# cv-core/MIT-Driverless-CV-TrainingInfra

Measured on AMD Instinct MI355X. Metric: images/sec training (YOLOv3 416^2 + RektNet 80^2), higher is better.
Workload: dtype bf16; 1 GPU; CVC-YOLOv3 yolo_baseline 416x416 classes=80, train step (fwd+bwd+Adam), 32 img/GPU; global_batch=32, parallelism=dp1, hipgraph=False, optimizer=FusedAdam

## Files before the change

### include/mdcv_hip.h

```cpp
#ifndef MDCV_HIP_H
#define MDCV_HIP_H
#ifdef __cplusplus
extern "C" {
#endif

#define MDCV_OK 0
#define MDCV_EARG (-1)
#define MDCV_F32 0
#define MDCV_BF16 1
#define MDCV_TUNED(dtype, code) (((dtype) & 0xff) | ((code) * 256))
#define MDCV_ACT_NONE 0
#define MDCV_ACT_LEAKY 1
#define MDCV_ACT_RELU 2

int mdcv_conv2d(int dtype, int mode, const void* in, int in_ldc, const void* w_packed, void* out, int out_ldc,
                const float* bias, const void* addsrc, int add_ldc, float* stats_partial,
                int B, int Hin, int Win, int Cin, int Hout, int Wout, int Nout,
                int KH, int KW, int stride, int pad, int dil, void* stream);
int mdcv_conv2d_affine_act(int dtype, const void* in, int in_ldc, const void* w_packed, void* out, int out_ldc, const float* scale,
                           const float* shift, const void* addsrc, int add_ldc, int act, float slope, int B, int Hin, int Win, int Cin,
                           int Hout, int Wout, int Nout, int KH, int KW, int stride, int pad, int dil, void* stream);
int mdcv_conv2d_dgrad_bnsums_rows(int dtype, int B, int Hin, int Win, int Cin, int Hout, int Wout, int Nout, int KH, int KW, int stride,
                                  int pad, int dil, int in_ldc);
int mdcv_conv2d_dgrad_bnsums(int dtype, const void* in, int in_ldc, const void* w_packed, void* out, int out_ldc, const void* addsrc,
                             int add_ldc, int B, int Hin, int Win, int Cin, int Hout, int Wout, int Nout, int KH, int KW, int stride,
                             int pad, int dil, const void* y, int ldy, const float* scale, const float* shift, const float* mean, int act,
                             float slope, float* partial, void* stream);
int mdcv_first_conv_ok(int dtype, int B, int H, int W, int Cin_pad, int Cout_pad, int KH, int KW, int stride, int pad, int dil, int ldx);
int mdcv_first_conv_rows(int B, int H);
int mdcv_first_conv_stats(int dtype, const void* x, int ldx, const void* w_packed, float* partial, int B, int H, int W, void* stream);
int mdcv_first_conv_bn_act(int dtype, const void* x, int ldx, const void* w_packed, const float* scale, const float* shift, int act, float slope,
                           void* y, int ldy, void* z, int ldz, int B, int H, int W, void* stream);
int mdcv_conv2d_dgrad_s2_form_ok(int dtype, int B, int Hin, int Win, int Cin, int Hout, int Wout, int Nout, int KH, int KW, int stride,
                                 int pad, int dil, int in_ldc);
int mdcv_xstats_words(int reps, int C);
int mdcv_xstats_reps(int rows, int C);
int mdcv_conv2d_xstats(int dtype, const void* in, int in_ldc, const void* w_packed, void* out, int out_ldc, const float* bias, void* xacc,
                       int reps, int B, int Hin, int Win, int Cin, int Hout, int Wout, int Nout, int KH, int KW, int stride, int pad, int dil,
                       void* stream);
int mdcv_pw_conv_fwd_xstats(int dtype, const void* y, int ldy, const float* scale, const float* shift, const void* resid, int ldr, int act,
                            float slope, void* z_out, int ldz, const void* w_packed, const float* bias, void* out, int out_ldc, void* xacc,
                            int reps, long long M, int K, int N, void* stream);
int mdcv_bn_act_fwd_xstats(int dtype, const void* y, int ldy, const void* xacc, int reps, double count, const float* gamma, const float* beta,
                           float* running_mean, float* running_var, float momentum, float eps, float* scale, float* shift, float* mean,
                           float* invstd, const void* resid, int ldr, void* out, int ldo, int M, int C, int act, float slope, void* stream);
int mdcv_conv2d_stats_rows(int M);
int mdcv_conv2d_stats_rows_geom(int dtype, int B, int Hout, int Wout, int Cin, int Nout, int KH, int KW, int stride, int pad, int dil,
                                int in_ldc);

int mdcv_conv2d_wgrad_splits(int dtype, int M, int Cout, int Ktot);
int mdcv_conv2d_wgrad_splits_geom(int dtype, int B, int Hin, int Win, int Cin, int Hout, int Wout, int Cout, int KH, int KW, int stride,
                                  int pad, int dil, int dy_ldc, int x_ldc);
int mdcv_conv2d_wgrad(int dtype, const void* dy, int dy_ldc, const void* x, int x_ldc, float* ws, int splits,
                      float* dw_oihw, int accumulate, int B, int Hin, int Win, int Cin, int Cin_real,
                      int Hout, int Wout, int Cout, int Cout_real, int KH, int KW, int stride, int pad, int dil, void* stream);

int mdcv_pack_weights(int dtype, const float* w_oihw, void* w_fwd, void* w_dgrad, int Cout, int Cin, int KH, int KW,
                      int Cout_pad, int Cin_pad, void* stream);

int mdcv_pack_weights_batched(int dtype, const void* table, int nlayers, int max_taps, void* stream);

int mdcv_nchw_to_nhwc(int dtype, const float* src, void* dst, int B, int C, int H, int W, int ldc, int Cpad, void* stream);
int mdcv_nhwc_to_nchw(int dtype, const void* src, int ldc, float* dst, int B, int C, int H, int W, void* stream);

int mdcv_partial_reduce(const float* partial, int rows, int nsums, int C, double* accum, void* stream);
int mdcv_bn_finalize(double* accum, double count, const float* gamma, const float* beta, float* running_mean, float* running_var,
                     float momentum, float eps, float* scale, float* shift, float* mean, float* invstd, int C, void* stream);
int mdcv_bn_eval_coeffs(const float* gamma, const float* beta, const float* running_mean, const float* running_var, float eps,
                        float* scale, float* shift, int C, void* stream);
int mdcv_bn_eval_coeffs_bias(const float* gamma, const float* beta, const float* running_mean, const float* running_var, float eps,
                             const float* conv_bias, float* scale, float* shift, int C, void* stream);
int mdcv_bn_act_fwd(int dtype, const void* y1, int ld1, const float* s1, const float* b1, const void* y2, int ld2, const float* s2,
                    const float* b2, const void* resid, int ldr, void* out, int ldo, int M, int C, int act, float slope, void* stream);
int mdcv_bn_act_bwd_reduce_ws_floats(int dtype, int M, int C, int nsums);
int mdcv_bn_stats_finalize(const float* partial, int rows, double* accum, double count, const float* gamma, const float* beta,
                           float* running_mean, float* running_var, float momentum, float eps, float* scale, float* shift, float* mean,
                           float* invstd, int C, void* stream);
int mdcv_bn_act_bwd_reduce_finalize(int dtype, const void* dout, int ldd, const void* y1, int ld1, const float* s1, const float* b1,
                                    const float* mean1, const float* invstd1, const void* y2, int ld2, const float* s2, const float* b2,
                                    const float* mean2, const float* invstd2, float* partial_ws, int M, int C, int act, float slope,
                                    double count, const float* gamma1, float* dgamma1, float* dbeta1, float* cA1, float* cB1, float* cC1,
                                    const float* gamma2, float* dgamma2, float* dbeta2, float* cA2, float* cB2, float* cC2, void* stream);
int mdcv_bn_bwd_finalize_rows(const float* partial, int rows, int C, double count, const float* gamma, const float* mean,
                              const float* invstd, float* dgamma, float* dbeta, float* cA, float* cB, float* cC, void* stream);
int mdcv_bn_act_bwd_reduce(int dtype, const void* dout, int ldd, const void* y1, int ld1, const float* s1, const float* b1,
                           const float* mean1, const float* invstd1, const void* y2, int ld2, const float* s2, const float* b2,
                           const float* mean2, const float* invstd2, double* accum, float* partial_ws, int M, int C, int act, float slope,
// ... 174 lines not shown
```

### mit-driverless-cv-traininginfra_amd/csrc/bn_fuse.h

```cpp
#pragma once
#include "common.h"

struct EpiArgs { const float* oscale; int act; float slope; };

struct BnFuseArgs {
  const void* y;
  const float* scale; const float* shift; const float* mean;
  float* partial;
  int ldy, act, row_base;
  float slope;
};

__device__ __forceinline__ void lds_only_barrier() { asm volatile("s_waitcnt lgkmcnt(0)\n\ts_barrier" ::: "memory"); }

__device__ __forceinline__ float swap_add16(float u, float v) {
  const auto r = __builtin_amdgcn_permlane16_swap(__builtin_bit_cast(unsigned, u), __builtin_bit_cast(unsigned, v), false, false);
  return __builtin_bit_cast(float, (unsigned)r[0]) + __builtin_bit_cast(float, (unsigned)r[1]);
}
__device__ __forceinline__ float swap_add32(float u, float v) {
  const auto r = __builtin_amdgcn_permlane32_swap(__builtin_bit_cast(unsigned, u), __builtin_bit_cast(unsigned, v), false, false);
  return __builtin_bit_cast(float, (unsigned)r[0]) + __builtin_bit_cast(float, (unsigned)r[1]);
}
template <int CTRL> __device__ __forceinline__ float ror_add(float x) {
  return x + __builtin_bit_cast(float, __builtin_amdgcn_update_dpp(0, __builtin_bit_cast(int, x), CTRL, 0xf, 0xf, false));
}

template <typename T, int BN, int NT>
struct BnFuseAcc {
  static constexpr int VEC = ET<T>::VEC;
  static constexpr int VPRO = BN / VEC;
  static constexpr int RPP = NT / VPRO;
  static_assert(NT % VPRO == 0 && RPP <= 128 && 128 % RPP == 0 && VPRO <= 64, "store-loop geometry");
  float fs[VEC], fb[VEC], fm[VEC], sg[VEC], sx[VEC];

  __device__ __forceinline__ void init(const BnFuseArgs& f, int n0, int Nout) {
#pragma unroll
    for (int e = 0; e < VEC; ++e) {
      const bool ok = f.y && n0 + e < Nout;
      fs[e] = ok ? f.scale[n0 + e] : 0.f; fb[e] = ok ? f.shift[n0 + e] : 0.f; fm[e] = ok ? f.mean[n0 + e] : 0.f;
      sg[e] = 0.f; sx[e] = 0.f;
    }
  }
  __device__ __forceinline__ void add(const BnFuseArgs& f, const float (&dv)[VEC], const uint4& yq) {
    float yv[VEC];
    ET<T>::unpack(yq, yv);
#pragma unroll
    for (int e = 0; e < VEC; ++e) {
      const float pre = __builtin_fmaf(yv[e], fs[e], fb[e]);
      const float g = (f.act != 0 && !(pre > 0.f)) ? dv[e] * f.slope : dv[e];
      sg[e] += g;
      sx[e] += g * (yv[e] - fm[e]);
    }
  }
  static constexpr bool kWaveFold = VEC == 8 && VPRO <= 16;
  static constexpr int WROWS = 64 / VPRO;
  __device__ __forceinline__ void fold_wave(float* ws, int lane) {
    float w[8], x[4];
#pragma unroll
    for (int m = 0; m < 4; ++m) { w[m] = swap_add16(sg[2 * m], sg[2 * m + 1]); w[4 + m] = swap_add16(sx[2 * m], sx[2 * m + 1]); }
#pragma unroll
    for (int n = 0; n < 4; ++n) x[n] = swap_add32(w[2 * n], w[2 * n + 1]);
#pragma unroll
    for (int n = 0; n < 4; ++n) {
      if constexpr (VPRO <= 8) x[n] = ror_add<0x128>(x[n]);
      if constexpr (VPRO <= 4) x[n] = ror_add<0x124>(x[n]);
      if constexpr (VPRO <= 2) x[n] = ror_add<0x122>(x[n]);
    }
    const int rho = lane >> 4, c16 = lane & 15;
    if (c16 < VPRO) {
      float* r0 = ws + c16 * VEC + rho;
      r0[0] = x[0]; r0[4] = x[1]; r0[BN] = x[2]; r0[BN + 4] = x[3];
    }
#pragma unroll
    for (int e = 0; e < VEC; ++e) { sg[e] = 0.f; sx[e] = 0.f; }
  }
  static __device__ __forceinline__ void write_row(const BnFuseArgs& f, const float* ws0, int wstride, int t, int n_tile0, int Nout, int row) {
    const int which = t / BN, c = t - which * BN;
    float tot = 0.f;
#pragma unroll
    for (int wv = 0; wv < NT / 64; ++wv) tot += ws0[wv * wstride + t];
    const int n = n_tile0 + c;
    if (n < Nout) f.partial[(size_t)(f.row_base + row) * 2 * Nout + (size_t)which * Nout + n] = tot;
  }

  __device__ __forceinline__ void flush(const BnFuseArgs& f, float* red, int tid, int n_tile0, int Nout, int row) {
    const int lane = tid & 63, wave = tid >> 6;
    {
#pragma unroll
      for (int off = 32; off >= VPRO; off >>= 1) {
#pragma unroll
        for (int e = 0; e < VEC; ++e) { sg[e] += __shfl_xor(sg[e], off, 64); sx[e] += __shfl_xor(sx[e], off, 64); }
      }
      float tot[2] = {0.f, 0.f};
#pragma unroll
      for (int k = 0; k < 2; ++k) {
        if (lane < VPRO) {
#pragma unroll
          for (int e = 0; e < VEC; ++e) red[wave * BN + lane * VEC + e] = k == 0 ? sg[e] : sx[e];
        }
        lds_only_barrier();
        if (tid < BN) {
#pragma unroll
          for (int w = 0; w < NT / 64; ++w) tot[k] += red[w * BN + tid];
        }
// ... 16 lines not shown
```

### mit-driverless-cv-traininginfra_amd/csrc/conv_igemm.hip

```cpp
#include "conv_gemm.h"
#include "conv_shift.h"
#include "wgrad_gemm.h"
#include "wgrad_shift.h"
#include "wgrad_stream.h"

extern "C" {

static int conv2d_impl(int dtype, int mode, const void* in, int in_ldc, const void* w_packed, void* out, int out_ldc,
                       const float* bias, const void* addsrc, int add_ldc, float* stats_partial,
                       int B, int Hin, int Win, int Cin, int Hout, int Wout, int Nout,
                       int KH, int KW, int stride, int pad, int dil, const BnFuseArgs* fuse, void* stream, const EpiArgs* epi = nullptr,
                       const XAccArgs* xacc = nullptr) {
  if (!in || !w_packed || !out) return MDCV_EARG;
  if (xacc && (mode != 0 || stats_partial || fuse || epi || !xacc->acc || xacc->reps < 1 || (xacc->reps & (xacc->reps - 1)))) return MDCV_EARG;
  if (epi && (mode != 0 || stats_partial || fuse)) return MDCV_EARG;
  if ((Cin & 7) || (Nout & 7) || (in_ldc & 7) || (out_ldc & 7) || (addsrc && (add_ldc & 7))) return MDCV_EARG;
  if (stride != 1 && stride != 2) return MDCV_EARG;
  if (mode != 0 && mode != 1) return MDCV_EARG;
  ConvArgs a;
  a.in = in; a.w = w_packed; a.out = out; a.bias = bias; a.addsrc = addsrc; a.stats = stats_partial;
  a.in_ldc = in_ldc; a.out_ldc = out_ldc; a.add_ldc = add_ldc;
  a.Hin = Hin; a.Win = Win; a.Cin = Cin; a.Hout = Hout; a.Wout = Wout; a.Nout = Nout;
  a.KH = KH; a.KW = KW; a.stride = stride; a.pad = pad; a.dil = dil;
  a.M = B * Hout * Wout; a.Ktot = KH * KW * Cin; a.tiles_n = 0; a.sshift = stride == 2 ? 1 : 0; a.tiles_total = 0; a.xcd_chunk = 0;
// ... 85 lines not shown
                           int Hout, int Wout, int Nout, int KH, int KW, int stride, int pad, int dil, void* stream) {
  MDCV_TUNE_ENTRY(dtype, MDCV_TUNE_CONV);
  if (act < 0 || act > 2) return MDCV_EARG;
  const EpiArgs e{scale, act, slope};
  return conv2d_impl(dtype, 0, in, in_ldc, w_packed, out, out_ldc, shift, addsrc, add_ldc, nullptr, B, Hin, Win, Cin, Hout, Wout, Nout,
                     KH, KW, stride, pad, dil, nullptr, stream, &e);
}

int mdcv_conv2d_dgrad_bnsums_rows(int dtype, int B, int Hin, int Win, int Cin, int Hout, int Wout, int Nout, int KH, int KW, int stride,
                                  int pad, int dil, int in_ldc) {
  MDCV_TUNE_ENTRY(dtype, MDCV_TUNE_CONV);
  const int es = 2;
  if (dtype != MDCV_BF16) return 0;
  if (!conv_operands_small((long long)B * Hin * Win * in_ldc * es, (long long)Nout * KH * KW * Cin * es)) return 0;
  if (Hin == Hout && Win == Wout && mdcv_shift_eligible(dtype, B, Hout, Wout, Cin, Nout, KH, KW, stride, pad, dil, in_ldc))
    return mdcv_shift_stats_rows(B, Hout, Wout, dil, Nout);
  if (stride == 2 && dil == 1 && KH == 3 && KW == 3 && pad == 1 && Hout == 2 * Hin && Wout == 2 * Win && TUNE().conv_variant < 0 &&
      mdcv_shift_s2_dgrad_eligible(dtype, B, Hin, Win, Cin, Nout, in_ldc))
    return mdcv_shift_s2_rows(B, Hin, Win);
  if (stride == 2 && dil == 1) {
    int rows = 0;
    for (int cls = 0; cls < 4; ++cls) {
      const int ph = cls >> 1, pw = cls & 1;
      const int m = B * ((Hout - ph + 1) / 2) * ((Wout - pw + 1) / 2);
      if (m > 0) rows += cdiv(m, 128);
    }
    return rows;
  }
  return cdiv(B * Hout * Wout, 128);
}

int mdcv_conv2d_dgrad_bnsums(int dtype, const void* in, int in_ldc, const void* w_packed, void* out, int out_ldc, const void* addsrc,
                             int add_ldc, int B, int Hin, int Win, int Cin, int Hout, int Wout, int Nout, int KH, int KW, int stride,
                             int pad, int dil, const void* y, int ldy, const float* scale, const float* shift, const float* mean, int act,
                             float slope, float* partial, void* stream) {
  MDCV_TUNE_ENTRY(dtype, MDCV_TUNE_CONV);
  if (!y || !scale || !shift || !mean || !partial || (ldy & 7)) return MDCV_EARG;
  if (mdcv_conv2d_dgrad_bnsums_rows(dtype, B, Hin, Win, Cin, Hout, Wout, Nout, KH, KW, stride, pad, dil, in_ldc) <= 0) return MDCV_EARG;
  BnFuseArgs f;
  f.y = y; f.scale = scale; f.shift = shift; f.mean = mean; f.partial = partial; f.ldy = ldy; f.act = act; f.row_base = 0;
  f.slope = act == 2 ? 0.f : slope;
  return conv2d_impl(dtype, 1, in, in_ldc, w_packed, out, out_ldc, nullptr, addsrc, add_ldc, nullptr, B, Hin, Win, Cin, Hout, Wout, Nout,
                     KH, KW, stride, pad, dil, &f, stream);
}

int mdcv_conv2d_dgrad_s2_form_ok(int dtype, int B, int Hin, int Win, int Cin, int Hout, int Wout, int Nout, int KH, int KW, int stride,
                                 int pad, int dil, int in_ldc) {
  MDCV_TUNE_ENTRY(dtype, MDCV_TUNE_CONV);
  return dtype == MDCV_BF16 && stride == 2 && dil == 1 && KH == 3 && KW == 3 && pad == 1 && Hout == 2 * Hin && Wout == 2 * Win &&
         TUNE().conv_variant < 0 && (long long)B * Hin * Win * in_ldc * 2 < (1LL << 31) &&
         mdcv_shift_s2_dgrad_eligible(dtype, B, Hin, Win, Cin, Nout, in_ldc);
}

int mdcv_conv2d_stats_rows(int M) { return cdiv(M, 128); }
int mdcv_conv2d_stats_rows_geom(int dtype, int B, int Hout, int Wout, int Cin, int Nout, int KH, int KW, int stride, int pad, int dil,
                                int in_ldc) {
  MDCV_TUNE_ENTRY(dtype, MDCV_TUNE_CONV);
  if (mdcv_shift_eligible(dtype, B, Hout, Wout, Cin, Nout, KH, KW, stride, pad, dil, in_ldc)) return mdcv_shift_fwd_stats_rows(B, Hout, Wout, Nout, dil);
  return cdiv(B * Hout * Wout, 128);
}

int mdcv_conv2d_wgrad_splits(int dtype, int M, int Cout, int Ktot) {
  MDCV_TUNE_ENTRY(dtype, MDCV_TUNE_WGRAD);
  const int bp = dtype == MDCV_BF16 ? 128 : 64;
  const int tiles = cdiv(Cout, 128) * cdiv(Ktot, 128);
  const int slots = TUNE().wgrad_slots;
  int s = slots / tiles;
  const int max_s = cdiv(M, bp * 4);
  if (s > max_s) s = max_s;
  if (s < 1) s = 1;
  int pps = cdiv(cdiv(M, s), bp) * bp;
  return cdiv(M, pps);
}

enum WgradFamily { WG_STEM, WG_STREAM, WG_SHIFT, WG_S2, WG_GENERIC };

static bool wgrad_eligible(WgradFamily f, const WgradGeom& g) {
  const int v = TUNE().wgrad_variant;
  if (f == WG_GENERIC) return true;
  if (v == 9 || (v == 10 && f != WG_SHIFT)) return false;
  const bool same = g.Hin == g.Hout && g.Win == g.Wout;
  switch (f) {
    case WG_STEM:
      return same && mdcv_wgrad_stem_eligible(g.dtype, g.B, g.Hout, g.Wout, g.Cin, g.Cout, g.KH, g.KW, g.stride, g.pad, g.dil, g.dy_ldc, g.x_ldc);
    case WG_STREAM:
      return same && mdcv_wgrad_stream_eligible(g.dtype, g.B, g.Hout, g.Wout, g.Cin, g.Cout, g.KH, g.KW, g.stride, g.pad, g.dil, g.dy_ldc, g.x_ldc);
    case WG_S2:
      return mdcv_wgrad_s2_eligible(g.dtype, g.B, g.Hin, g.Win, g.Cin, g.Hout, g.Wout, g.Cout, g.KH, g.KW, g.stride, g.pad, g.dil, g.dy_ldc, g.x_ldc);
    default: break;
  }
  if (!same || !mdcv_wgrad_shift_eligible(g.dtype, g.B, g.Hout, g.Wout, g.Cin, g.Cout, g.KH, g.KW, g.stride, g.pad, g.dil, g.dy_ldc, g.x_ldc)) return false;
  if (v == 8) return true;
  const long long Mq = (long long)g.B * (g.Hout + 1) * (g.Wout + 1);
  const int s = mdcv_wgrad_shift_splits(g.B, g.Hout, g.Wout, g.Cin, g.Cout);
  if (Mq / (64LL * s) >= 128) return true;
  return v == 11 && mdcv_conv2d_wgrad_splits(g.dtype, g.B * g.Hout * g.Wout, g.Cout, g.KH * g.KW * g.Cin) == 1;
}

static int wgrad_family_splits(WgradFamily f, const WgradGeom& g) {
  switch (f) {
    case WG_STEM:   return mdcv_wgrad_stem_splits(g.B, g.Hout, g.Wout);
    case WG_STREAM: return mdcv_wgrad_stream_splits(g.B, g.Hout, g.Wout, g.Cin, g.Cout, g.dil);
    case WG_SHIFT:  return mdcv_wgrad_shift_splits(g.B, g.Hout, g.Wout, g.Cin, g.Cout);
    case WG_S2:     return mdcv_wgrad_s2_splits(g.B, g.Hout, g.Wout, g.Cin, g.Cout);
    default:        return mdcv_conv2d_wgrad_splits(g.dtype, g.B * g.Hout * g.Wout, g.Cout, g.KH * g.KW * g.Cin);
  }
// ... 72 lines not shown
```

### mit-driverless-cv-traininginfra_amd/csrc/conv_shift.h

```cpp
#pragma once
#include <hip/hip_runtime.h>
#include "bn_fuse.h"
#include "exact_acc.h"

struct ShiftArgs {
  const void* in; const void* w; void* out; const float* bias; const void* addsrc; float* stats;
  int in_ldc, out_ldc, add_ldc;
  int B, H, W, Cin, Nout;
  int Wq, Sq, Mq;
  int tiles_n, tiles_total, xcd_chunk;
  int p_base;
  int dil;
  BnFuseArgs fuse;
  EpiArgs epi;
  int t2d, tiles_x, tiles_y, TH;
  int nchunks, wrow, nca;
  XAccArgs xacc;
};

bool mdcv_shift_eligible(int dtype, int B, int H, int W, int Cin, int Nout, int KH, int KW, int stride, int pad, int dil, long long in_ldc);
int mdcv_shift_stats_rows(int B, int H, int W, int dil = 1, int Nout = 128);
int mdcv_shift_fwd_stats_rows(int B, int H, int W, int Nout, int dil = 1);
int mdcv_shift_conv(int mode, const void* in, int in_ldc, const void* w, void* out, int out_ldc, const float* bias, const void* addsrc,
                    int add_ldc, float* stats, int B, int H, int W, int Cin, int Nout, const BnFuseArgs* fuse, hipStream_t st,
                    const EpiArgs* epi = nullptr, int dil = 1, const XAccArgs* xacc = nullptr);
int mdcv_shift_s2_rows(int B, int H, int W);
bool mdcv_shift_s2_dgrad_eligible(int dtype, int B, int H, int W, int Cin, int Nout, long long in_ldc);
```

### mit-driverless-cv-traininginfra_amd/csrc/conv_shift.hip

```cpp
#include "common.h"
#include "conv_shift.h"
#include "bn_fuse.h"

#ifndef MDCV_SHIFT_PART
#define MDCV_SHIFT_PART 0
#endif
#if MDCV_SHIFT_PART == 0
#else
#endif
int mdcv_shift_launch_dgrad(const ShiftArgs& a, hipStream_t st, unsigned in_bytes, unsigned w_bytes);

namespace {

[[maybe_unused]] constexpr int BN = 128;
constexpr int WM = 4;
constexpr unsigned OOB = 0x80000000u;

__device__ __forceinline__ int swz(int row) { return (row >> 1) & 2; }
typedef __attribute__((address_space(3))) void lds_void_t;

#if defined(MDCV_SHIFT_TS) || defined(MDCV_SHIFT_WG)
#include <cstdio>
__device__ long long g_shift_wg[3 * 4096];
#endif
// ... 239 lines not shown
    bf16_t* __restrict__ out3 = reinterpret_cast<bf16_t*>(a.out);
    const bf16_t* __restrict__ add3 = reinterpret_cast<const bf16_t*>(a.addsrc);
    constexpr int VPRO3 = BN / 8;
    static_assert((512 * VPRO3) % (NW * 64) == 0 && (NW * 64) % VPRO3 == 0, "every thread keeps one channel vector");
    using Acc3 = BnFuseAcc<bf16_t, BN, NW * 64>;
    Acc3 fz3;
    const bf16_t* __restrict__ fy3 = reinterpret_cast<const bf16_t*>(a.fuse.y);
    if constexpr (FUSE) fz3.init(a.fuse, tile_n * BN + (tid % VPRO3) * 8, a.Nout);
#pragma unroll
    for (int py = 0; py < 2; ++py) {
#pragma unroll
      for (int px = 0; px < 2; ++px)
#pragma unroll
        for (int i = 0; i < FM; ++i)
#pragma unroll
          for (int j = 0; j < FN; ++j)
#pragma unroll
            for (int rr = 0; rr < 4; ++rr) {
              const int p = wm * TM + i * 16 + (lane >> 4) * 4 + rr, col = wn * TN + j * 16 + (lane & 15);
              const int srow = (p >> 5) * 64 + 2 * (p & 31) + px;
              reinterpret_cast<bf16_t*>(smem + srow * SROW)[col] = f2bf(acc[(2 * py + px) * FM + i][j][rr]);
            }
      __syncthreads();
      long long pixv[VPRO3]; uint4 aq[VPRO3], yq[VPRO3];
      const int cv = tid % VPRO3, n = tile_n * BN + cv * 8;
#pragma unroll
      for (int k = 0; k < VPRO3; ++k) {
        const int srow = (tid + k * NW * 64) / VPRO3;
        const int la = srow >> 6, ox = srow & 63;
        const int Y = 2 * (a0 + la) + py, X = 2 * b0 + ox;
        const bool ok = ox < 2 * (a.Wq - 1) && Y < Ho && X < Wo && n < a.Nout;
        pixv[k] = ok ? ((long long)img * Ho + Y) * Wo + X : -1;
        if (ok) {
          if (add3) aq[k] = *reinterpret_cast<const uint4*>(add3 + pixv[k] * a.add_ldc + n);
          if constexpr (FUSE) yq[k] = *reinterpret_cast<const uint4*>(fy3 + pixv[k] * a.fuse.ldy + n);
        }
      }
#pragma unroll
      for (int k = 0; k < VPRO3; ++k) {
        if (pixv[k] >= 0) {
          const int srow = (tid + k * NW * 64) / VPRO3;
          uint4 d = *reinterpret_cast<const uint4*>(smem + srow * SROW + cv * 16);
          float x[8];
          if (add3 || FUSE) ET<bf16_t>::unpack(d, x);
          if (add3) {
            float y[8];
            ET<bf16_t>::unpack(aq[k], y);
#pragma unroll
            for (int e = 0; e < 8; ++e) x[e] += y[e];
            d = ET<bf16_t>::pack(x);
            if constexpr (FUSE) ET<bf16_t>::unpack(d, x);
          }
          if constexpr (FUSE) {
            fz3.add(a.fuse, x, yq[k]);
          }
          *reinterpret_cast<uint4*>(out3 + pixv[k] * a.out_ldc + n) = d;
        }
      }
      __syncthreads();
    }
    if constexpr (FUSE) {
      static_assert(Acc3::kWaveFold, "bf16, at most 16 channel vectors per pixel");
      float* ws3 = reinterpret_cast<float*>(smem + 512 * SROW);
      fz3.fold_wave(ws3 + wave * 2 * BN, lane);
      lds_only_barrier();
      for (int t = tid; t < 2 * BN; t += NW * 64) Acc3::write_row(a.fuse, ws3, 2 * BN, t, tile_n * BN, a.Nout, tile_m);
    }
    return;
  }
  int* rowpix = reinterpret_cast<int*>(smem + PIX_OFF);
  if (tid < BM) {
    int img, y, x;
    bool ok;
    if (a.t2d) {
      const int tpi = a.tiles_x * a.tiles_y;
      img = tile_m / tpi;
      const int rt = tile_m - img * tpi, ty = rt / a.tiles_x, tx = rt - ty * a.tiles_x;
      const int ly = tid / a.Wq, lx = tid - ly * a.Wq;
      y = ty * a.TH + ly; x = tx * (a.Wq - 2) + lx;
      ok = lx < a.Wq - 2 && ly < a.TH;
    } else {
      const int p = p0 + tid;
      ok = p < a.Mq;
      const int pp = ok ? p : 0;
      img = pp / a.Sq;
      const int rem = pp - img * a.Sq;
      y = rem / a.Wq; x = rem - y * a.Wq;
    }
    ok = ok && y < a.H && x < a.W;
    rowpix[tid] = ok ? (img * a.H + y) * a.W + x : -1;
  }
  const int n0 = tile_n * BN + wn * TN;
  if constexpr (EPI) {
#pragma unroll
    for (int j = 0; j < FN; ++j) {
      const int n = n0 + j * 16 + (lane & 15);
      const float sc = (a.epi.oscale && n < a.Nout) ? a.epi.oscale[n] : 1.f;
      const float bv = (a.bias && n < a.Nout) ? a.bias[n] : 0.f;
      const float sl = a.epi.act == 1 ? a.epi.slope : (a.epi.act == 2 ? 0.f : 1.f);
#pragma unroll
      for (int i = 0; i < FM; ++i)
#pragma unroll
        for (int rr = 0; rr < 4; ++rr) {
          const float v = acc[i][j][rr] * sc + bv;
          acc[i][j][rr] = v > 0.f ? v : v * sl;
        }
    }
// ... 211 lines not shown
  return launch_shift<MODE, BM, 5, 2, BN_>(a, p_base, tiles_m, st, in_bytes, w_bytes);
}

int shift_plan_bm(int Mq, int tiles_n, bool fused, int halo = 0, int bn = 128, bool fwd = false) {
  if (halo > 0 && !fused && 2 * ((256 + halo + 15) / 16) * 1024 + 3 * bn * 64 + 1024 > 80 * 1024) {
    for (int bm = 256; bm >= 128; bm -= 64) {
      const int nca = (bm + halo + 15) / 16;
      if (2 * nca * 1024 + 3 * bn * 64 + 1024 <= 80 * 1024) return bm;
    }
    return 256;
  }
  if (bn == 128 && !fused && fwd && halo <= 110) {
    const int t384 = ((Mq + 383) / 384) * tiles_n;
    if (TUNE().shift_big == 384 || (TUNE().shift_loop == 2 && t384 > 192 && t384 <= 256)) return 384;
  }
  if (TUNE().shift_plan == 1) return 256;
  if (TUNE().shift_plan == 2) return 128;
  const int t256 = ((Mq + 255) / 256) * tiles_n;
  if (t256 <= 128) return 128;
  if (fused || TUNE().shift_plan == 6) return 256;
  const int t192 = ((Mq + 191) / 192) * tiles_n;
  const int c256 = ((t256 + 255) / 256) * 256, c192 = ((t192 + 255) / 256) * 192;
  return c192 < c256 ? 192 : 256;
}

template <int MODE, int BN_>
int launch_shift_mode(const ShiftArgs& a, hipStream_t st, unsigned in_bytes, unsigned w_bytes) {
  if constexpr (MODE == 3) {
    return launch_shift_bm<MODE, 256, BN_>(a, 0, a.Mq / 256, st, in_bytes, w_bytes);
  } else {
  if (a.t2d) return launch_shift_bm<MODE, 256, BN_>(a, 0, a.Mq / 256, st, in_bytes, w_bytes);
  const int bm = shift_plan_bm(a.Mq, a.tiles_n, a.fuse.y != nullptr, 2 * a.dil * (a.Wq + 1), BN_, MODE == 0);
  if constexpr (BN_ == 128 && MODE == 0) {
    if (bm == 384) return launch_shift_bm<MODE, 384, BN_>(a, 0, (a.Mq + 383) / 384, st, in_bytes, w_bytes);
  }
  if (bm == 192) return launch_shift_bm<MODE, 192, BN_>(a, 0, (a.Mq + 191) / 192, st, in_bytes, w_bytes);
  const int big_m = (a.Mq + 255) / 256;
  const int nbig_m = bm == 128 ? 0 : big_m;
  if (nbig_m > 0) {
    const int rc = launch_shift_bm<MODE, 256, BN_>(a, 0, nbig_m, st, in_bytes, w_bytes);
    if (rc) return rc;
  }
  const int p_base = nbig_m * 256;
  if (p_base < a.Mq) return launch_shift_bm<MODE, 128, BN_>(a, p_base, (a.Mq - p_base + 127) / 128, st, in_bytes, w_bytes);
  return MDCV_OK;
  }
}

}

#if MDCV_SHIFT_PART == 1
int mdcv_shift_launch_dgrad(const ShiftArgs& a, hipStream_t st, unsigned in_bytes, unsigned w_bytes) {
  if (a.t2d == 2) {
    if (a.Nout == 32) return launch_shift_mode<3, 32>(a, st, in_bytes, w_bytes);
    if (a.Nout == 64) return launch_shift_mode<3, 64>(a, st, in_bytes, w_bytes);
    return MDCV_EARG;
  }
  if (a.Nout == 32) return launch_shift_mode<1, 32>(a, st, in_bytes, w_bytes);
  if (a.Nout == 64) return launch_shift_mode<1, 64>(a, st, in_bytes, w_bytes);
  if (TUNE().shift_n64_wide && !a.t2d && a.Nout % 64 == 0 && ((a.Mq + 255) / 256) * a.tiles_n <= 128) {
    ShiftArgs b = a;
    b.tiles_n = a.Nout / 64;
    return launch_shift_mode<1, 64>(b, st, in_bytes, w_bytes);
  }
  return launch_shift_mode<1, 128>(a, st, in_bytes, w_bytes);
}
#else
static bool shift_fits_1d(int W, int Nout) {
  return W <= TUNE().shift_wmax || (TUNE().shift_wmax_narrow && Nout <= 64 && W <= TUNE().shift_wmax_narrow) || (TUNE().shift_wmax_n32 && Nout <= 32 && W <= TUNE().shift_wmax_n32);
}
static bool shift_is_2d(int W, int Nout, int dil) { return dil == 1 && TUNE().shift_2d && !shift_fits_1d(W, Nout); }
constexpr int T2D_WQ = 32, T2D_TH = 8;
static long long shift_2d_positions(int B, int H, int W) { return (long long)B * ((H + T2D_TH - 1) / T2D_TH) * ((W + T2D_WQ - 3) / (T2D_WQ - 2)) * 256; }

bool mdcv_shift_eligible(int dtype, int B, int H, int W, int Cin, int Nout, int KH, int KW, int stride, int pad, int dil, long long in_ldc) {
  if (dtype != MDCV_BF16 || KH != 3 || KW != 3 || stride != 1 || pad != dil || (dil != 1 && !(dil == 2 && TUNE().shift_dil2))) return false;
  if (dil == 2 && TUNE().shift_dil2 == 1 && !(Nout <= 64 && Cin >= 64)) return false;
  if ((Cin & 31) || ((Nout & 127) && !(Nout == 64 && TUNE().shift_n64) && !(Nout == 32 && TUNE().shift_n64 == 2))) return false;
  if (H < 8 || W < 8) return false;
  if (!shift_fits_1d(W, Nout) && !(TUNE().shift_2d && dil == 1)) return false;
  if ((long long)B * (H + dil) * (W + dil) + 1024 >= (1LL << 30) || shift_2d_positions(B, H, W) >= (1LL << 30)) return false;
  if ((long long)B * H * W * in_ldc * 2 >= (1LL << 31) || (long long)Nout * 9 * Cin * 2 >= (1LL << 31)) return false;
  return true;
}

bool mdcv_shift_s2_dgrad_eligible(int dtype, int B, int H, int W, int Cin, int Nout, long long in_ldc) {
  if (!TUNE().shift_s2 || dtype != MDCV_BF16 || (Cin & 31) || Cin < 32 || !(Nout == 32 || Nout == 64) || H < 1 || W < 1) return false;
  if ((long long)B * ((H + 7) / 8) * ((W + 30) / 31) * 256 >= (1LL << 30)) return false;
  if ((long long)B * H * W * in_ldc * 2 >= (1LL << 31) || (long long)Nout * 9 * Cin * 2 >= (1LL << 31)) return false;
  return true;
}

int mdcv_shift_s2_rows(int B, int H, int W) { return B * ((H + T2D_TH - 1) / T2D_TH) * ((W + T2D_WQ - 2) / (T2D_WQ - 1)); }

int mdcv_shift_stats_rows(int B, int H, int W, int dil, int Nout) {
  if (shift_is_2d(W, Nout, dil)) return (int)(shift_2d_positions(B, H, W) / 128);
  return (int)(((long long)B * (H + dil) * (W + dil) + 127) / 128);
}
int mdcv_shift_fwd_stats_rows(int B, int H, int W, int Nout, int dil) {
  if (shift_is_2d(W, Nout, dil)) return (int)(shift_2d_positions(B, H, W) / 128);
  const int Mq = B * (H + dil) * (W + dil);
  const int bn = Nout <= 64 ? Nout : BN;
  const int bm = shift_plan_bm(Mq, Nout <= 64 ? 1 : Nout / BN, false, 2 * dil * (W + dil + 1), bn, true);
  return (bm == 192 || bm == 384) ? (Mq + bm - 1) / bm : (Mq + 127) / 128;
}

// ... 58 lines not shown
```

### mit-driverless-cv-traininginfra_amd/csrc/tune.h

```cpp
#pragma once

struct MdcvTune {
  int conv_no_ut = 0;
  int conv_tall_narrow = 256;
  int conv_deep_narrow = 1;
  int conv_deep_small = 8;
  int conv_fuse_narrow = 1;
  int conv_variant = -1;
  int conv_tall_s2 = 1;
  int conv_deep_s2 = 1;
  int conv_s2_allcls = 1;
  int conv_s2_split = 512;
  int conv_s2_split_on = 1;
  int wgrad_slots = 512;
  int wgrad_bna_stages = 2;
  int wgrad_variant = 0;
  int shift_ring = 4;
  int shift_wmax_narrow = 104;
  int shift_wmax_n32 = 0;
  int shift_dil2 = 1;
  int shift_n64 = 2;
  int shift_wmax = 80;
  int shift_loop = 2;
  int shift_2d = 1;
  int shift_big = 0;
  int shift_n64_wide = 1;
  int shift_plan = 0;
  int shift_s2 = 1;
  int pw_bmp = 0;
  int pw_wres = 1;
  int stream_blocks = 0;
  int stream_tiled = 1;
  int stream_light_maxpos = 600000;
  int stream_table = 1;
  int stream_direct = 1;
  int stream_s2 = 1;
  int stream_s2_blocks = 256;
  int stream_s2_depth = 2;
  int stream_s2_lds = 160 * 1024;
  int stream_light_depth = 1;
  int stream_light_blocks = 256;
  int stream_tiled_blocks = 128;
};

extern thread_local const MdcvTune* mdcv_t_tune;
inline const MdcvTune& TUNE() { return *mdcv_t_tune; }

enum { MDCV_TUNE_CONV = 0, MDCV_TUNE_WGRAD = 1, MDCV_TUNE_PW = 2 };

inline void mdcv_tune_shift(MdcvTune& t, int ring) {
  if (ring == 63 || ring == 64) { t.shift_n64_wide = ring - 63; return; }
  if (ring == 29 || ring == 60) { t.shift_s2 = ring == 60; return; }
  if (ring == 27 || ring == 28) { t.shift_2d = ring - 27; return; }
  if (ring >= 200 && ring < 300) { t.shift_big = ring == 201 ? 384 : 0; return; }
  if (ring >= 30 && ring <= 59) { t.shift_loop = ring - 30; return; }
  if (ring == 25 || ring == 26) { t.shift_wmax_n32 = ring == 25 ? 208 : 0; return; }
  if (ring == 23 || ring == 24) { t.shift_wmax_narrow = ring == 23 ? 104 : 0; return; }
  if (ring >= 20 && ring <= 22) { t.shift_dil2 = ring == 20 ? 2 : (ring == 21 ? 0 : 1); return; }
  if (ring >= 17 && ring <= 19) { t.shift_n64 = ring == 17 ? 1 : (ring == 18 ? 0 : 2); return; }
  if (ring >= 14 && ring <= 16) { t.shift_wmax = ring == 14 ? 80 : (ring == 15 ? 62 : 104); return; }
  if (ring >= 7) t.shift_plan = ring - 7;
  else if (ring >= 3 && ring <= 5) t.shift_ring = ring;
}
inline void mdcv_tune_apply_conv(MdcvTune& t, int v) {
  if (v == 0) return;
  if (v <= -3 && v >= -299) { mdcv_tune_shift(t, -v); return; }
  if (v == 93 || v == 92) { t.conv_fuse_narrow = v == 93; return; }
  if (v >= 60 && v < 92) { t.conv_deep_small = v - 60; return; }
  if (v >= 30 && v < 60) { t.conv_deep_narrow = v - 30; return; }
  if (v == 20 || v == 21) { t.conv_deep_s2 = v - 20; return; }
  if (v == 16 || v == 17) { t.conv_s2_allcls = v - 16; return; }
  if (v == 14 || v == 15) { t.conv_s2_split_on = v - 14; return; }
  if (v >= 4000 && v < 6000) { t.conv_s2_split = v - 4000; return; }
  if (v == 18 || v == 19) { t.conv_tall_s2 = v - 18; return; }
  if (v >= 2000 && v < 3000) { t.conv_tall_narrow = v - 2000; return; }
  if (v >= 100) { t.conv_no_ut = 1; v -= 100; }
  if (v >= 1 && v <= 12) t.conv_variant = v - 1;
}
inline void mdcv_tune_apply_wgrad(MdcvTune& t, int v) {
  if (v == 0) return;
  if (v >= 20000 && v < 30000) { t.wgrad_slots = v - 20000; return; }
  if (v >= 35000 && v < 36000) { t.stream_s2_blocks = v - 35000; return; }
  if (v >= 30000 && v < 40000) {
    const int b = v - 30000;
    if (b >= 4001 && b <= 4002) { t.stream_light_depth = b - 4000; return; }
    if (b >= 4012 && b <= 4014) { t.wgrad_bna_stages = b - 4010; return; }
    if (b == 4020 || b == 4021) { t.stream_table = b - 4020; return; }
    if (b == 4050 || b == 4051) { t.stream_direct = b - 4050; return; }
    if (b == 4060 || b == 4061) { t.stream_s2 = b - 4060; return; }
    if (b >= 4071 && b <= 4073) { t.stream_s2_depth = b - 4070; return; }
    if (b >= 4100 && b <= 4260) { t.stream_s2_lds = (b - 4100) * 1024; return; }
    if (b == 2) t.stream_light_maxpos = 600000;
    else if (b == 3) t.stream_light_maxpos = 1 << 30;
    else if (b == 5) t.stream_light_maxpos = 0;
    else if (b >= 3000 && b < 4000) t.stream_light_blocks = b - 3000;
    else t.stream_tiled_blocks = b > 0 ? b : 128;
    return;
  }
  if (v >= 1000) { const int d = (v - 1000) / 100; t.stream_tiled = !(d & 8); t.stream_blocks = ((v - 1000) % 100) * 64; return; }
  t.wgrad_variant = v;
}
inline void mdcv_tune_apply_pw(MdcvTune& t, int v) {
  if (v == 1000 || v == 1001) { t.pw_wres = v - 1000; return; }
  if (v == 64 || v == 32 || v == 16) t.pw_bmp = v;
}

struct TuneScope {
  MdcvTune t;
  const MdcvTune* prev;
  int dtype;
  TuneScope(int dtype_arg, int family) : prev(mdcv_t_tune), dtype(dtype_arg & 0xff) {
    const int code = dtype_arg >> 8;
    if (code != 0) {
      if (family == MDCV_TUNE_CONV) mdcv_tune_apply_conv(t, code);
      else if (family == MDCV_TUNE_WGRAD) mdcv_tune_apply_wgrad(t, code);
      else mdcv_tune_apply_pw(t, code);
      mdcv_t_tune = &t;
    }
  }
// ... 7 lines not shown
```

Baseline: 2501 images/sec.

## Add persistent stride-2 shift dgrad kernel with cross-tile prefetch

```diff
diff --git a/include/mdcv_hip.h b/include/mdcv_hip.h
--- a/include/mdcv_hip.h
+++ b/include/mdcv_hip.h
@@ -33,6 +33,7 @@
                            void* y, int ldy, void* z, int ldz, int B, int H, int W, void* stream);
 int mdcv_conv2d_dgrad_s2_form_ok(int dtype, int B, int Hin, int Win, int Cin, int Hout, int Wout, int Nout, int KH, int KW, int stride,
                                  int pad, int dil, int in_ldc);
+int mdcv_conv2d_dgrad_s2_persistent(int dtype, int Nout);
 int mdcv_xstats_words(int reps, int C);
 int mdcv_xstats_reps(int rows, int C);
 int mdcv_conv2d_xstats(int dtype, const void* in, int in_ldc, const void* w_packed, void* out, int out_ldc, const float* bias, void* xacc,
diff --git a/mit-driverless-cv-traininginfra_amd/csrc/bn_fuse.h b/mit-driverless-cv-traininginfra_amd/csrc/bn_fuse.h
--- a/mit-driverless-cv-traininginfra_amd/csrc/bn_fuse.h
+++ b/mit-driverless-cv-traininginfra_amd/csrc/bn_fuse.h
@@ -50,6 +50,17 @@
       const float g = (f.act != 0 && !(pre > 0.f)) ? dv[e] * f.slope : dv[e];
       sg[e] += g;
       sx[e] += g * (yv[e] - fm[e]);
+    }
+  }
+  __device__ __forceinline__ void add_fma(const BnFuseArgs& f, const float (&dv)[VEC], const uint4& yq) {
+    float yv[VEC];
+    ET<T>::unpack(yq, yv);
+#pragma unroll
+    for (int e = 0; e < VEC; ++e) {
+      const float pre = __builtin_fmaf(yv[e], fs[e], fb[e]);
+      const float g = (f.act != 0 && !(pre > 0.f)) ? dv[e] * f.slope : dv[e];
+      sg[e] += g;
+      sx[e] = __builtin_fmaf(g, yv[e] - fm[e], sx[e]);
     }
   }
   static constexpr bool kWaveFold = VEC == 8 && VPRO <= 16;
diff --git a/mit-driverless-cv-traininginfra_amd/csrc/conv_igemm.hip b/mit-driverless-cv-traininginfra_amd/csrc/conv_igemm.hip
--- a/mit-driverless-cv-traininginfra_amd/csrc/conv_igemm.hip
+++ b/mit-driverless-cv-traininginfra_amd/csrc/conv_igemm.hip
@@ -161,6 +161,11 @@
          mdcv_shift_s2_dgrad_eligible(dtype, B, Hin, Win, Cin, Nout, in_ldc);
 }
 
+int mdcv_conv2d_dgrad_s2_persistent(int dtype, int Nout) {
+  MDCV_TUNE_ENTRY(dtype, MDCV_TUNE_CONV);
+  return dtype == MDCV_BF16 && TUNE().shift_s2 && mdcv_shift_s2_persistent(Nout) ? 1 : 0;
+}
+
 int mdcv_conv2d_stats_rows(int M) { return cdiv(M, 128); }
 int mdcv_conv2d_stats_rows_geom(int dtype, int B, int Hout, int Wout, int Cin, int Nout, int KH, int KW, int stride, int pad, int dil,
                                 int in_ldc) {
diff --git a/mit-driverless-cv-traininginfra_amd/csrc/conv_shift.h b/mit-driverless-cv-traininginfra_amd/csrc/conv_shift.h
--- a/mit-driverless-cv-traininginfra_amd/csrc/conv_shift.h
+++ b/mit-driverless-cv-traininginfra_amd/csrc/conv_shift.h
@@ -26,3 +26,5 @@
                     const EpiArgs* epi = nullptr, int dil = 1, const XAccArgs* xacc = nullptr);
 int mdcv_shift_s2_rows(int B, int H, int W);
 bool mdcv_shift_s2_dgrad_eligible(int dtype, int B, int H, int W, int Cin, int Nout, long long in_ldc);
+bool mdcv_shift_s2_persistent(int Nout);
+int mdcv_shift_s2p_launch(const ShiftArgs& a, hipStream_t st, unsigned in_bytes, unsigned w_bytes);
diff --git a/mit-driverless-cv-traininginfra_amd/csrc/conv_shift.hip b/mit-driverless-cv-traininginfra_amd/csrc/conv_shift.hip
--- a/mit-driverless-cv-traininginfra_amd/csrc/conv_shift.hip
+++ b/mit-driverless-cv-traininginfra_amd/csrc/conv_shift.hip
@@ -315,7 +315,7 @@
             if constexpr (FUSE) ET<bf16_t>::unpack(d, x);
           }
           if constexpr (FUSE) {
-            fz3.add(a.fuse, x, yq[k]);
+            fz3.add_fma(a.fuse, x, yq[k]);
           }
           *reinterpret_cast<uint4*>(out3 + pixv[k] * a.out_ldc + n) = d;
         }
@@ -633,6 +633,7 @@
 #if MDCV_SHIFT_PART == 1
 int mdcv_shift_launch_dgrad(const ShiftArgs& a, hipStream_t st, unsigned in_bytes, unsigned w_bytes) {
   if (a.t2d == 2) {
+    if (mdcv_shift_s2_persistent(a.Nout)) return mdcv_shift_s2p_launch(a, st, in_bytes, w_bytes);
     if (a.Nout == 32) return launch_shift_mode<3, 32>(a, st, in_bytes, w_bytes);
     if (a.Nout == 64) return launch_shift_mode<3, 64>(a, st, in_bytes, w_bytes);
     return MDCV_EARG;
diff --git a/mit-driverless-cv-traininginfra_amd/csrc/conv_shift_s2p.hip b/mit-driverless-cv-traininginfra_amd/csrc/conv_shift_s2p.hip
--- /dev/null
+++ b/mit-driverless-cv-traininginfra_amd/csrc/conv_shift_s2p.hip
@@ -0,0 +1,331 @@
+#include "common.h"
+#include "conv_shift.h"
+#include "bn_fuse.h"
+
+namespace {
+
+constexpr unsigned OOB = 0x80000000u;
+__device__ __forceinline__ int swz(int row) { return (row >> 1) & 2; }
+typedef __attribute__((address_space(3))) void lds_void_t;
+template <int N> __device__ __forceinline__ void wait_vm() { asm volatile("s_waitcnt vmcnt(%0)" ::"n"(N) : "memory"); }
+template <int N> __device__ __forceinline__ void wait_vm_reads_done() { asm volatile("s_waitcnt vmcnt(%0) lgkmcnt(0)" ::"n"(N) : "memory"); }
+
+template <int BN> struct S2pGeom {
+  static constexpr int NW = 8, WN = 2, NPA = 3, NCA = 21;
+  static constexpr int BTILE = BN * 64, SROW = BN * 2 + 16, ABYTES = NCA * 1024;
+  static constexpr int STG = 512 * SROW;
+  static constexpr int EXTRA = ((STG - ABYTES + 1023) / 1024) * 1024;
+  static constexpr int A1OFF = ABYTES + EXTRA, BBASE = A1OFF + ABYTES, SINK = BBASE + 3 * BTILE;
+  static constexpr int WS_OFF = SINK + 1024, TAB_OFF = WS_OFF + NW * 2 * BN * 4, LDS = TAB_OFF + 3 * BN * 4;
+  static constexpr int WPC = BN == 32 ? 2 : 1;
+  static_assert(EXTRA >= 0 && A1OFF >= STG && EXTRA + ABYTES >= STG, "the staging area fits beside the buffer the prefetch lands in");
+};
+
+}
+
+template <int BN_, bool FUSE>
+__global__ __launch_bounds__(512) __attribute__((amdgpu_waves_per_eu(BN_ == 32 ? 4 : 2, BN_ == 32 ? 4 : 2)))
+void mdcv_shift_s2p_kernel(ShiftArgs a, unsigned in_bytes, unsigned w_bytes, int lanes, int grid) {
+  using G = S2pGeom<BN_>;
+  constexpr int BN = BN_, BTILE = G::BTILE, SROW = G::SROW, NW = G::NW, WN = G::WN, NPA = G::NPA, ABYTES = G::ABYTES;
+  constexpr int TN = BN / WN, FN = TN / 16, TM = 64, FM = 4, LA = 2, BRING = 3;
+  extern __shared__ __attribute__((aligned(1024))) unsigned char smem[];
+
+  const int x = (int)blockIdx.x % lanes, jx = (int)blockIdx.x / lanes, nx = (grid - x + lanes - 1) / lanes;
+  const int hi = min((x + 1) * a.xcd_chunk, a.tiles_total);
+  int t = x * a.xcd_chunk + jx;
+  if (t >= hi) return;
+
+  const int tid = threadIdx.x;
+  const int wave = __builtin_amdgcn_readfirstlane(tid >> 6);
+  const int wm = wave / WN, wn = wave % WN;
+  const int tpi = a.tiles_x * a.tiles_y;
+
+  const __amdgpu_buffer_rsrc_t rin = __builtin_amdgcn_make_buffer_rsrc(const_cast<void*>(a.in), 0, in_bytes, 0x00020000);
+  const __amdgpu_buffer_rsrc_t rw = __builtin_amdgcn_make_buffer_rsrc(const_cast<void*>(a.w), 0, w_bytes, 0x00020000);
+#define S2P_ABUF(B) ((B) ? G::A1OFF : 0)
+#define S2P_ISSUE_A(RS, AVO, CHUNK, BUF)                                                                               \
+  do {                                                                                                                \
+    const int base__ = S2P_ABUF(BUF);                                                                                 \
+    const int so__ = (CHUNK) * 64;                                                                                    \
+    _Pragma("unroll") for (int k = 0; k < NPA; ++k) {                                                                 \
+      const int ch__ = wave + k * NW;              \
+      __builtin_amdgcn_raw_ptr_buffer_load_lds(RS, (lds_void_t*)(smem + (ch__ < G::NCA ? base__ + ch__ * 1024 : G::SINK)), 16, \
+                                               (int)(AVO)[k], so__, 0, 0);                                            \
+    }                                                                                                                 \
+  } while (0)
+#define S2P_ISSUE_B(RS, TAP, CHUNK, SLOT)                                                                             \
+  __builtin_amdgcn_raw_ptr_buffer_load_lds(RS, (lds_void_t*)(smem + (wave < BN / 16 ? G::BBASE + (SLOT) * BTILE + wave * 1024 : G::SINK)), 16, \
+                                           (int)bvo, ((TAP) * a.Cin + (CHUNK) * 32) * 2, 0, 0)
+
+  const int Ho = 2 * a.H, Wo = 2 * a.W;
+  bf16_t* __restrict__ out3 = reinterpret_cast<bf16_t*>(a.out);
+  const bf16_t* __restrict__ add3 = reinterpret_cast<const bf16_t*>(a.addsrc);
+  const bf16_t* __restrict__ fy3 = reinterpret_cast<const bf16_t*>(a.fuse.y);
+  constexpr int VPRO3 = BN / 8;
+  using Acc3 = BnFuseAcc<bf16_t, BN, NW * 64>;
+  static_assert(Acc3::kWaveFold, "bf16, at most 16 channel vectors per pixel");
+  Acc3 fz3;
+  float* ws3 = reinterpret_cast<float*>(smem + G::WS_OFF);
+  float* tab = reinterpret_cast<float*>(smem + G::TAB_OFF);
+  const volatile f32x4_t* tabv = reinterpret_cast<const volatile f32x4_t*>(smem + G::TAB_OFF);
+  if constexpr (FUSE) {
+    if (tid < BN) {
+      const bool ok = tid < a.Nout;
+      tab[tid] = ok ? a.fuse.scale[tid] : 0.f; tab[BN + tid] = ok ? a.fuse.shift[tid] : 0.f; tab[2 * BN + tid] = ok ? a.fuse.mean[tid] : 0.f;
+    }
+  }
+
+  const int nch = a.nchunks;
+  int par = 0;
+  bool first = true;
+  for (;;) {
+    const int tnext = t + nx;
+    const bool has_next = tnext < hi;
+    int ktid = tid;
+    asm volatile("" : "+v"(ktid));
+    const int lane = ktid & 63, lrow = lane >> 2, kv = (lane & 3) ^ swz(lrow);
+    auto tile_avo = [&](int tile, unsigned (&av)[NPA]) {
+      const int img = tile / tpi, rt = tile - img * tpi, ty = rt / a.tiles_x, tx = rt - ty * a.tiles_x;
+#pragma unroll
+      for (int k = 0; k < NPA; ++k) {
+        const int j = (wave + k * NW) * 16 + lrow;
+        const int yy = ty * 8 + (j >> 5), xx = tx * 31 + (j & 31);
+        const bool ok = yy < a.H && xx < a.W && kv * 8 < a.Cin;
+        av[k] = ok ? (unsigned)((((img * a.H + yy) * a.W + xx) * a.in_ldc + kv * 8) * 2) : OOB;
+      }
+    };
+    const unsigned bvo = (wave < BN / 16 && wave * 16 + lrow < a.Nout) ? (unsigned)(((wave * 16 + lrow) * a.wrow + kv * 8) * 2) : OOB;
+    const int r = lane & 15, q = lane >> 4;
+    int offA[9];
+#pragma unroll
+    for (int tap = 0; tap < 9; ++tap) {
+      const int kh = tap / 3, kw = tap - kh * 3;
+      const int row = wm * TM + (kh == 0 ? 32 : 0) + (kw == 0 ? 1 : 0) + r;
+      offA[tap] = row * 64 + ((q ^ swz(row)) << 4);
+    }
+    const int offB = (wn * TN + r) * 64 + ((q ^ swz(r)) << 4);
+    unsigned avo[NPA], avn[NPA];
+    tile_avo(t, avo);
+    if (first) {
+      S2P_ISSUE_A(rin, avo, 0, 0);
+      S2P_ISSUE_B(rw, 0, 0, 0);
+      S2P_ISSUE_B(rw, 1, 0, 1);
+      first = false;
+    }
+    tile_avo(has_next ? tnext : t, avn);
+    const __amdgpu_buffer_rsrc_t rinN = __builtin_amdgcn_make_buffer_rsrc(const_cast<void*>(a.in), 0, has_next ? in_bytes : 0u, 0x00020000);
+    const __amdgpu_buffer_rsrc_t rwN = __builtin_amdgcn_make_buffer_rsrc(const_cast<void*>(a.w), 0, has_next ? w_bytes : 0u, 0x00020000);
+
+    f32x4_t acc[4 * FM][FN];
+#pragma unroll
+    for (int i = 0; i < 4 * FM; ++i)
+#pragma unroll
+      for (int j = 0; j < FN; ++j) acc[i][j] = f32x4_t{0.f, 0.f, 0.f, 0.f};
+#define S2P_TAP_CLS(T) (((((T) / 3) != 1 ? 2 : 0) + (((T) % 3) != 1 ? 1 : 0)) * FM)
+
+    for (int c0 = 0; c0 < nch; c0 += 2) {
+#pragma unroll
+      for (int cc = 0; cc < 2; ++cc) {
+        const int c = c0 + cc;
+        if (c < nch) {
+          const bool lastc = c == nch - 1;
+          const int abase = S2P_ABUF((cc & 1) ^ par);
+#pragma unroll
+          for (int tap = 0; tap < 9; ++tap) {
+            const int rslot = (cc * 9 + tap) % BRING, wslot = (cc * 9 + tap + LA) % BRING;
+#pragma unroll
+            for (int i = 0; i < 4 * FM; ++i)
+#pragma unroll
+              for (int j = 0; j < FN; ++j) asm volatile("" : "+v"(acc[i][j]));
+            if (tap >= 1 && tap <= LA) wait_vm_reads_done<LA - 1 + NPA>(); else wait_vm_reads_done<LA - 1>();
+            __builtin_amdgcn_s_barrier();
+            bf16x8_t fa[FM], fb[FN];
+            const unsigned char* pa = smem + abase + offA[tap];
+            const unsigned char* pb = smem + G::BBASE + rslot * BTILE + offB;
+#pragma unroll
+            for (int i = 0; i < FM; ++i) fa[i] = *reinterpret_cast<const bf16x8_t*>(pa + i * 1024);
+#pragma unroll
+            for (int j = 0; j < FN; ++j) fb[j] = *reinterpret_cast<const bf16x8_t*>(pb + j * 1024);
+            {
+              const int t2 = (tap + LA) % 9, c2 = c + (tap + LA) / 9;
+              if (tap + LA >= 9 && lastc) S2P_ISSUE_B(rwN, t2, 0, wslot);
+              else S2P_ISSUE_B(rw, t2, c2, wslot);
+            }
+            if (tap == 0) {
+              if (lastc) S2P_ISSUE_A(rinN, avn, 0, ((cc + 1) & 1) ^ par);
+              else S2P_ISSUE_A(rin, avo, c + 1, ((cc + 1) & 1) ^ par);
+            }
+#pragma unroll
+            for (int i = 0; i < FM; ++i)
+#pragma unroll
+              for (int j = 0; j < FN; ++j)
+                acc[S2P_TAP_CLS(tap) + i][j] = __builtin_amdgcn_mfma_f32_16x16x32_bf16(fa[i], fb[j], acc[S2P_TAP_CLS(tap) + i][j], 0, 0, 0);
+          }
+        }
+      }
+    }
+    const int lastbuf = ((nch - 1) & 1) ^ par;
+    unsigned char* stg = smem + (lastbuf ? ABYTES : 0);
+
+    unsigned pk[4][FM][FN][2];
+#pragma unroll
+    for (int s4 = 0; s4 < 4; ++s4)
+#pragma unroll
+      for (int i = 0; i < FM; ++i)
+#pragma unroll
+        for (int j = 0; j < FN; ++j) {
+          pk[s4][i][j][0] = pack_bf16x2(acc[s4 * FM + i][j][0], acc[s4 * FM + i][j][1]);
+          pk[s4][i][j][1] = pack_bf16x2(acc[s4 * FM + i][j][2], acc[s4 * FM + i][j][3]);
+          asm volatile("" : "+v"(pk[s4][i][j][0]), "+v"(pk[s4][i][j][1])::"memory");
+        }
+    const int img = t / tpi, rt = t - img * tpi, ty = rt / a.tiles_x, tx = rt - ty * a.tiles_x;
+    const int a0 = ty * 8, b0 = tx * 31;
+    if constexpr (FUSE) {
+#pragma unroll
+      for (int e = 0; e < 8; ++e) { fz3.sg[e] = 0.f; fz3.sx[e] = 0.f; }
+    }
+    int elane = 0;
+#pragma unroll
+    for (int py = 0; py < 2; ++py) {
+      int pixv[VPRO3]; uint4 aq[VPRO3], yq[VPRO3];
+      {
+        int ltid = ktid;
+        asm volatile("" : "+v"(ltid));
+        const int n = (ltid % VPRO3) * 8;
+#pragma unroll
+        for (int k = 0; k < VPRO3; ++k) {
+          const int srow = (ltid + k * NW * 64) / VPRO3;
+          const int la = srow >> 6, ox = srow & 63;
+          const int Y = 2 * (a0 + la) + py, X = 2 * b0 + ox;
+          const bool ok = ox < 62 && Y < Ho && X < Wo && n < a.Nout;
+          pixv[k] = ok ? (img * Ho + Y) * Wo + X : -1;
+          const long long pl = ok ? pixv[k] : 0;
+          if (add3) aq[k] = *reinterpret_cast<const uint4*>(add3 + pl * a.add_ldc + n);
+          if constexpr (FUSE) yq[k] = *reinterpret_cast<const uint4*>(fy3 + pl * a.fuse.ldy + n);
+        }
+      }
+      lds_only_barrier();
+      {
+        int stid = ktid;
+        asm volatile("" : "+v"(stid));
+        const int sl = stid & 63;
+#pragma unroll
+        for (int px = 0; px < 2; ++px)
+#pragma unroll
+          for (int i = 0; i < FM; ++i)
+#pragma unroll
+            for (int j = 0; j < FN; ++j)
+#pragma unroll
+              for (int rr = 0; rr < 4; ++rr) {
+                const int p = wm * TM + i * 16 + (sl >> 4) * 4 + rr, col = wn * TN + j * 16 + (sl & 15);
+                const int srow = (p >> 5) * 64 + 2 * (p & 31) + px;
+                reinterpret_cast<bf16_t*>(stg + srow * SROW)[col] = (bf16_t)((pk[2 * py + px][i][j][rr >> 1] >> ((rr & 1) * 16)) & 0xffffu);
+              }
+      }
+      lds_only_barrier();
+      int etid = ktid;
+      asm volatile("" : "+v"(etid));
+      elane = etid & 63;
+      const int cv = etid % VPRO3, n = cv * 8;
+#pragma unroll
+      for (int k = 0; k < VPRO3; ++k) {
+        if (pixv[k] >= 0) {
+          const int srow = (etid + k * NW * 64) / VPRO3;
+          uint4 d = *reinterpret_cast<const uint4*>(stg + srow * SROW + cv * 16);
+          float xv[8];
+          if (add3 || FUSE) ET<bf16_t>::unpack(d, xv);
+          if (add3) {
+            float yv[8];
+            ET<bf16_t>::unpack(aq[k], yv);
+#pragma unroll
+            for (int e = 0; e < 8; ++e) xv[e] += yv[e];
+            d = ET<bf16_t>::pack(xv);
+            if constexpr (FUSE) ET<bf16_t>::unpack(d, xv);
+          }
+          if constexpr (FUSE) {
+            float yv[8];
+            ET<bf16_t>::unpack(yq[k], yv);
+#pragma unroll
+            for (int h = 0; h < 2; ++h) {
+              const f32x4_t fsv = tabv[cv * 2 + h], fbv = tabv[BN / 4 + cv * 2 + h], fmv = tabv[2 * (BN / 4) + cv * 2 + h];
+#pragma unroll
+              for (int e4 = 0; e4 < 4; ++e4) {
+                const int e = h * 4 + e4;
+                const float pre = __builtin_fmaf(yv[e], fsv[e4], fbv[e4]);
+                const float g = (a.fuse.act != 0 && !(pre > 0.f)) ? xv[e] * a.fuse.slope : xv[e];
+                fz3.sg[e] += g;
+                fz3.sx[e] = __builtin_fmaf(g, yv[e] - fmv[e4], fz3.sx[e]);
+              }
+            }
+          }
+          *reinterpret_cast<uint4*>(out3 + (long long)pixv[k] * a.out_ldc + n) = d;
+        }
+      }
+    }
+    if constexpr (FUSE) {
+      fz3.fold_wave(ws3 + wave * 2 * BN, elane);
+      lds_only_barrier();
+      for (int u = tid; u < 2 * BN; u += NW * 64) Acc3::write_row(a.fuse, ws3, 2 * BN, u, 0, a.Nout, t);
+    }
+    if (!has_next) break;
+    t = tnext;
+    par = lastbuf ^ 1;
+  }
+  wait_vm<0>();
+#undef S2P_ABUF
+#undef S2P_ISSUE_A
+#undef S2P_ISSUE_B
+#undef S2P_TAP_CLS
+}
+
+namespace {
+
+int s2p_device_cus() {
+  static std::atomic<int> cus[64];
+  int dev = 0;
+  if (hipGetDevice(&dev) != hipSuccess || dev < 0 || dev >= 64) return 256;
+  int n = cus[dev].load(std::memory_order_relaxed);
+  if (!n) {
+    n = (hipDeviceGetAttribute(&n, hipDeviceAttributeMultiprocessorCount, dev) == hipSuccess && n >= 8) ? n : 256;
+    cus[dev].store(n, std::memory_order_relaxed);
+  }
+  return n;
+}
+
+template <int BN, bool FUSE>
+int launch_s2p(ShiftArgs a, hipStream_t st, unsigned in_bytes, unsigned w_bytes, int cap) {
+  using G = S2pGeom<BN>;
+  a.p_base = 0;
+  a.tiles_total = a.Mq / 256;
+  a.nca = G::NCA;
+  int grid = TUNE().shift_s2_persist == 3 ? a.tiles_total : G::WPC * s2p_device_cus();
+  if (cap > 0 && cap < grid) grid = cap;
+  if (grid > a.tiles_total) grid = a.tiles_total;
+  if (grid >= 8) grid &= ~7;
+  const int lanes = grid < 8 ? grid : 8;
+  a.xcd_chunk = (a.tiles_total + lanes - 1) / lanes;
+  static DynLds dyn_lds;
+  auto kern = mdcv_shift_s2p_kernel<BN, FUSE>;
+  if (hipError_t e = mdcv_dyn_lds(dyn_lds, reinterpret_cast<const void*>(kern), G::LDS); e != hipSuccess) return (int)e;
+  MDCV_LAUNCH(kern, dim3((unsigned)grid), dim3(512), G::LDS, st, a, in_bytes, w_bytes, lanes, grid);
+  MDCV_CHECK_LAUNCH();
+  return MDCV_OK;
+}
+
+}
+
+bool mdcv_shift_s2_persistent(int Nout) {
+  const int m = TUNE().shift_s2_persist;
+  if (m == 0 || !(Nout == 32 || Nout == 64)) return false;
+  if (m == 1 || m == 3) return true;
+  return Nout == 32;
+}
+
+int mdcv_shift_s2p_launch(const ShiftArgs& a, hipStream_t st, unsigned in_bytes, unsigned w_bytes) {
+  if (a.t2d != 2 || a.tiles_n != 1 || a.Wq != 32 || a.TH != 8 || a.Mq < 256) return MDCV_EARG;
+  const int cap = TUNE().shift_s2_wgcap;
+  if (a.Nout == 32) return a.fuse.y ? launch_s2p<32, true>(a, st, in_bytes, w_bytes, cap) : launch_s2p<32, false>(a, st, in_bytes, w_bytes, cap);
+  if (a.Nout == 64) return a.fuse.y ? launch_s2p<64, true>(a, st, in_bytes, w_bytes, cap) : launch_s2p<64, false>(a, st, in_bytes, w_bytes, cap);
+  return MDCV_EARG;
+}
diff --git a/mit-driverless-cv-traininginfra_amd/csrc/tune.h b/mit-driverless-cv-traininginfra_amd/csrc/tune.h
--- a/mit-driverless-cv-traininginfra_amd/csrc/tune.h
+++ b/mit-driverless-cv-traininginfra_amd/csrc/tune.h
@@ -27,6 +27,8 @@
   int shift_n64_wide = 1;
   int shift_plan = 0;
   int shift_s2 = 1;
+  int shift_s2_persist = 2;
+  int shift_s2_wgcap = 0;
   int pw_bmp = 0;
   int pw_wres = 1;
   int stream_blocks = 0;
@@ -49,6 +51,8 @@
 enum { MDCV_TUNE_CONV = 0, MDCV_TUNE_WGRAD = 1, MDCV_TUNE_PW = 2 };
 
 inline void mdcv_tune_shift(MdcvTune& t, int ring) {
+  if (ring > 400 && ring < 1000) { t.shift_s2_persist = 1; t.shift_s2_wgcap = ring - 400; return; }
+  if (ring >= 65 && ring <= 68) { t.shift_s2_persist = ring - 65; return; }
   if (ring == 63 || ring == 64) { t.shift_n64_wide = ring - 63; return; }
   if (ring == 29 || ring == 60) { t.shift_s2 = ring == 60; return; }
   if (ring == 27 || ring == 28) { t.shift_2d = ring - 27; return; }
@@ -64,7 +68,7 @@
 }
 inline void mdcv_tune_apply_conv(MdcvTune& t, int v) {
   if (v == 0) return;
-  if (v <= -3 && v >= -299) { mdcv_tune_shift(t, -v); return; }
+  if (v <= -3 && v >= -999) { mdcv_tune_shift(t, -v); return; }
   if (v == 93 || v == 92) { t.conv_fuse_narrow = v == 93; return; }
   if (v >= 60 && v < 92) { t.conv_deep_small = v - 60; return; }
   if (v >= 30 && v < 60) { t.conv_deep_narrow = v - 30; return; }
```

Result: no change. 2523 images/sec (median of 6 runs) (+0.9%).
